# cube1324/ppo.c

Hardware: AMD Instinct MI355X
Metric: PPO updates/sec + env-steps/sec on 4096×256 synthetic rollout, 1/2/4/8 MI355X (higher is better)
Workload: dtype fp32

## Files before the change

include/ppo_ext.h:

```cpp
#ifndef PPO_EXT_H
#define PPO_EXT_H

#include <stddef.h>
#include <stdint.h>

#ifdef __cplusplus
extern "C" {
#endif


int         ppo_device_count(void);
int         ppo_set_device(int device);
const char* ppo_last_error(void);
void        ppo_clear_error(void);
void        ppo_synchronize(void);
const char* ppo_build_info(void);
int         ppo_struct_sizes(long* out, int n);

void* ppo_dev_alloc(size_t bytes);
void  ppo_dev_free(void* p);
void  ppo_h2d(void* dst, const void* src, size_t bytes);
void  ppo_d2h(void* dst, const void* src, size_t bytes);
void  ppo_d2d(void* dst, const void* src, size_t bytes);
void  ppo_dev_memset(void* dst, int value, size_t bytes);
// ... 23 lines not shown

void ppo_read_stats(void* ppo, double* out, int n);
void ppo_reset_stats(void* ppo);

int    ppo_set_max_grad_norm(void* ppo, float max_norm);
float  ppo_get_max_grad_norm(void* ppo);
double ppo_grad_norm_device(const float* d_a, long na, const float* d_b, long nb);

int    ppo_set_target_kl(void* ppo, float target_kl);
float  ppo_get_target_kl(void* ppo);
int    ppo_kl_history(void* ppo, double* out, int n);
int    ppo_policy_kl_device(const float* d_mu, const float* d_log_std, const float* d_action, const float* d_old_lp,
                            int m, int A, float eps, double* out2);
int    ppo_set_value_clip(void* ppo, float eps_v);
float  ppo_get_value_clip(void* ppo);
int    ppo_value_clip_old_values(void* ppo, const float* d_v_old, long n);
int    ppo_value_clip_head_device(const float* d_y, const float* d_v_old, const int* d_rows, const float* d_tgt, int m,
                                  float eps_v, float* d_g, double* out3);
int    ppo_set_obs_norm(void* ppo, float clip);
float  ppo_get_obs_norm(void* ppo);
int    ppo_obs_norm_freeze(void* ppo, int frozen);
int    ppo_obs_norm_fold_buffer(void* ppo);
int    ppo_obs_norm_get_state(void* ppo, double* out, long n);
int    ppo_obs_norm_set_state(void* ppo, const double* in, long n);
int    ppo_obs_norm_affine(void* ppo, float* mean, float* rstd, int S);
int    ppo_obs_normalize_device(void* ppo, const float* d_in, float* d_out, long m);
int    ppo_obs_stats_device(const float* d_x, long n, int S, double* out);
long ppo_gae_state(double* welford, float* v, float* v_next, long n);
void ppo_set_step_limit(void* ppo, long max_value_steps, long max_policy_steps);

void ppo_sample_action_device(void* policy, float* d_state, float* d_action, float* d_log_prob, int m,
                              unsigned long long seed, unsigned long long offset);

void ppo_fill_synthetic(void* ppo, int n_envs, int horizon, unsigned long long seed, float p_terminate);

void ppo_rollout_device(void* ppo, int n_envs, int horizon, int env_kind, unsigned long long seed);

int ppo_nn_input_rows(void* nn, float* out, int m);

int ppo_set_compute_dtype(void* ppo, int dtype);
int nn_set_compute_dtype(void* nn, int dtype);

int    ppo_gemm_tune(int force_cfg, int splitk_target);
int    ppo_gemm_flags(int flags);
double ppo_bench_gemm(int op, int m, int n, int l, int iters, int cfg);
double ppo_bench_streams(int two, int steps, int B, int out);
int    ppo_gemm16_tune(int force_cfg);
double ppo_bench_gemm16(int op, int m, int n, int l, int iters, int cfg, int splitk_target);

int    ppo_gemm_f32_engine(int engine);
int    ppo_gemm16_dma(int on);
int    ppo_gemm16_tn_width(int bn);
int    ppo_gemm_x3_tune(int force_cfg, int splitk_target);
int    ppo_x3_stamps(unsigned long long* out, int n);
int    ppo_g16_stamps(unsigned long long* out, int n);
double ppo_bench_gemm_x3(int op, int m, int n, int l, int iters, int cfg, int splitk_target);

enum { PPO_K_GEMM = 0, PPO_K_GAE = 1, PPO_K_ADAM = 2, PPO_K_GATHER = 3, PPO_K_HEAD = 4,
       PPO_K_COMM = 5, PPO_K_OTHER = 6, PPO_K_COUNT = 7 };
void ppo_prof_enable(int stride);
void ppo_prof_reset(void);
void ppo_prof_read(double* out_ms, double* out_work, long* out_launches);
void ppo_prof_kernel_events(int on);
int  ppo_prof_shapes(long long* keys, double* ms, long* launches, double* work, int cap);
int  ppo_prof_shape_issued(const long long* keys, long* issued, int n);
void ppo_prof_counts(long* out_total);
void ppo_prof_issued_work(double* out_work);

#ifdef __cplusplus
}
#endif
#endif
```

ppo.c_amd/csrc/gemm_x3.hip:

```cpp
#include "dev.h"
#include "vclip.h"

#include <algorithm>
#include <type_traits>

namespace {

typedef float f32x4 __attribute__((ext_vector_type(4)));
typedef float f32x16 __attribute__((ext_vector_type(16)));
typedef unsigned u32x4 __attribute__((ext_vector_type(4)));
typedef unsigned u32x2 __attribute__((ext_vector_type(2)));
typedef short s16x4 __attribute__((ext_vector_type(4)));
typedef short s16x8 __attribute__((ext_vector_type(8)));
typedef __bf16 bf16x8 __attribute__((ext_vector_type(8)));

constexpr int BK = 16;
enum { OP_NT = 0, OP_NN = 1, OP_TN = 2 };

__device__ unsigned long long g_x3_stamps[8192 * 8];

struct X3Args {
    const float* A; const float* B; float* C;
    int M, N, K, lda, ldb, ldc;
    const float* bias; int relu;
    const int* ridx; float* acopy;
    unsigned* bits_out; const unsigned* bits_in; int wpr;
    float* gbias;
    int kchunk, splits, tiles_m, tiles_n;
    float* slab;
    const float* ydot;
    float* ypart;
    const float* fold_g;
    const float* fold_w;
    const unsigned* fold_bits;
    int fold_wpr;
    float* fold_gw;
    const float* vh_ypart; const float* vh_b; const float* vh_t;
    float* vh_y; float* vh_gb; float* vh_loss;
    int vh_slots;
    PhipVClip vh_vc;
    const float* red_slab; float* red_out;
    long red_n, red_stride;
    int red_splits, red_wgs, gemm_wgs;
    hipEvent_t ev_start, ev_stop;
};

template <int NTH>
__device__ __forceinline__ void x3_slab_reduce_block(const X3Args& a, int blk, float* part) {
    typedef float f32x4_ __attribute__((ext_vector_type(4)));
    constexpr int Q = 4, C = NTH / Q;
    const int c = threadIdx.x % C, q = threadIdx.x / C;
    const long n4 = (a.red_n + 3) >> 2, s4 = a.red_stride >> 2;
    const long i = (long)blk * C + c;
    const int per = (a.red_splits + Q - 1) / Q;
    const int s0 = q * per, s1 = min(a.red_splits, s0 + per);
    const f32x4_* __restrict__ sv = reinterpret_cast<const f32x4_*>(a.red_slab);
    f32x4_ acc = {0.f, 0.f, 0.f, 0.f};
    if (i < n4) {
#pragma unroll 8
        for (int sp = s0; sp < s1; ++sp) acc += sv[(long)sp * s4 + i];
    }
    f32x4_* pv = reinterpret_cast<f32x4_*>(part);
    if (q) pv[(q - 1) * C + c] = acc;
    __syncthreads();
    if (q == 0 && i < n4) {
#pragma unroll
        for (int v = 0; v < Q - 1; ++v) acc += pv[v * C + c];
        if (4 * i + 4 <= a.red_n) {
            reinterpret_cast<f32x4_*>(a.red_out)[i] = acc;
        } else {
            for (int e = 0; e < 4; ++e)
                if (4 * i + e < a.red_n) a.red_out[4 * i + e] = acc[e];
        }
    }
}

__device__ __forceinline__ unsigned pack2(float lo, float hi) {
    typedef __bf16 bf16x2 __attribute__((ext_vector_type(2)));
    bf16x2 p = {(__bf16)lo, (__bf16)hi};
    return __builtin_bit_cast(unsigned, p);
}
__device__ __forceinline__ float bf_lo(unsigned u) { return __builtin_bit_cast(float, u << 16); }
__device__ __forceinline__ float bf_hi(unsigned u) { return __builtin_bit_cast(float, u & 0xffff0000u); }

__device__ __forceinline__ unsigned pack2_opaque(float lo, float hi) {
    unsigned u = pack2(lo, hi);
    asm("" : "+v"(u));
    return u;
}

__device__ __forceinline__ void split4(f32x4 f, u32x2& p0, u32x2& p1, u32x2& p2) {
    const unsigned a0 = pack2_opaque(f[0], f[1]), b0 = pack2_opaque(f[2], f[3]);
    const float r0 = f[0] - bf_lo(a0), r1 = f[1] - bf_hi(a0);
    const float r2 = f[2] - bf_lo(b0), r3 = f[3] - bf_hi(b0);
    const unsigned a1 = pack2_opaque(r0, r1), b1 = pack2_opaque(r2, r3);
    p0 = u32x2{a0, b0};
// ... 256 lines not shown
                }
                if (BITS && r < 16) {
                    const int row = r0 + (r & 3) + 8 * (r >> 2);
                    if (row < a.M && c0 < a.N) a.bits_out[(long)row * a.wpr + (c0 >> 5)] = word;
                }
            }
            if constexpr (YD) ydot_block(yp, i);
        }
    };
    if (OP == OP_NT && a.bits_out) body(std::true_type{});
    else body(std::false_type{});
}

template <int OP, int BM, int BN, int WARPS_M, int NTH, int OCC, int KG, int ABL = 0, int FOLD = 0, int KB = BK>
__device__ __forceinline__ void x3_body(const X3Args& a, int b, int grid) {
    constexpr int NTG = NTH / KG;
    constexpr int NW = NTG / 64, WARPS_N = NW / WARPS_M;
    constexpr int WM = BM / WARPS_M, WN = BN / WARPS_N;
    constexpr int TM = WM / 32, TN = WN / 32;
    static_assert(TM >= 1 && TN >= 1 && WARPS_M * WARPS_N == NW, "wave tiling");
    static_assert(KG == 1 || OP == OP_TN, "k-groups: grad_W only");
    constexpr bool A_MN = OP == OP_TN, B_MN = OP != OP_NT;
    using SA = StageX3<BM, A_MN, NTG, KB>;
    using SB = StageX3<BN, B_MN, NTG, KB>;
    constexpr int BUF = SA::SIZE + SB::SIZE;
    constexpr int KH = KB / 16;

    constexpr int NS = 3;
    extern __shared__ __attribute__((aligned(16))) unsigned short lds[];

    if constexpr (OP == OP_NN) {
        if (a.red_wgs && b >= a.gemm_wgs) {
            x3_slab_reduce_block<NTH>(a, b - a.gemm_wgs, reinterpret_cast<float*>(lds));
            return;
        }
    }

    const int nwg = (OP == OP_NN && a.red_wgs) ? a.gemm_wgs : grid;
    const int xcd = b & 7, qq = nwg >> 3, rr = nwg & 7;
    const int t = (xcd < rr ? xcd * (qq + 1) : rr * (qq + 1) + (xcd - rr) * qq) + (b >> 3);
    const int tn = t % a.tiles_n;
    const int rest = t / a.tiles_n;
    const int tm = rest % a.tiles_m;
    const int m0 = tm * BM, n0 = tn * BN;
    const int kbeg = (rest / a.tiles_m) * a.kchunk;
    const int kend = min(a.K, kbeg + a.kchunk);

    const int tid = threadIdx.x, lane = tid & 63;
    const int grp = KG > 1 ? __builtin_amdgcn_readfirstlane(tid / NTG) : 0;
    const int lt = KG > 1 ? tid % NTG : tid;
    const int w = lt >> 6;
    const int wm = w / WARPS_N, wn = w % WARPS_N;
    auto stamp = [&](int slot) {
        if (tid == 0 && b < 8192) {
            g_x3_stamps[b * 8 + slot] = __builtin_amdgcn_s_memtime();
            if (slot == 0 || slot == 3) g_x3_stamps[b * 8 + 4 + slot / 3] = __builtin_amdgcn_s_memrealtime();
        }
    };
    if (ABL & 32) stamp(0);
    const int r = lane & 31, h = lane >> 5;

    f32x16 acc[TM][TN];
#pragma unroll
    for (int i = 0; i < TM; ++i)
#pragma unroll
        for (int j = 0; j < TN; ++j)
#pragma unroll
            for (int e = 0; e < 16; ++e) acc[i][j][e] = 0.f;

    SA sa;
    SB sb;
    sa.init(a.A, a.lda, OP == OP_NT ? a.ridx : nullptr, m0, a.M, lt);
    sb.init(a.B, a.ldb, nullptr, n0, a.N, lt);
    constexpr bool syn = OP != OP_NT && FOLD != 0;
    constexpr int FMA_ = !syn ? 0 : OP == OP_NN ? 2 : 1;
    constexpr int FMB_ = syn ? 1 : 0;
    const float* fold_g = a.fold_g;
    if constexpr (OP == OP_TN && FOLD != 0) {
        if (a.vh_ypart) {
            float* gl = reinterpret_cast<float*>(lds + KG * NS * BUF);
            const bool head = tm == 0 && tn == 0;
            const float bias = a.vh_b[0];
            float ls = 0.f, sgs = 0.f;
            int nclip = 0, nrow = 0;
            for (int rr = tid; rr < kend - kbeg; rr += NTH) {
                const int row = kbeg + rr;
                float yv = 0.f;
                for (int q = 0; q < a.vh_slots; ++q) yv += a.vh_ypart[(long)q * a.K + row];
                yv += bias;
                float gv;
                const float lv = ppo::value_head_row(yv, a.vh_t[row], (float)a.K, a.vh_vc, row, gv, nclip);
                gl[rr] = gv;
                if (head) {
                    a.vh_y[row] = yv;
                    const_cast<float*>(a.fold_g)[row] = gv;
                    ls += lv;
                    sgs += gv;
                    ++nrow;
                }
            }
            if (head) {
                ls = ppo::wave_sum64(ls);
                sgs = ppo::wave_sum64(sgs);
                if (lane == 0) {
                    atomicAdd(a.vh_gb, sgs);
                    if (a.vh_loss) atomicAdd(a.vh_loss, ls * (1.0f / (float)a.K));
                }
                if (a.vh_vc.v_old) {
                    const float fc = ppo::wave_sum64((float)nclip), fr = ppo::wave_sum64((float)nrow);
// ... 324 lines not shown
                        wv[e] = a.bits_in[(long)min(r0 + (e & 3) + 8 * (e >> 2), a.M - 1) * a.wpr + (c0 >> 5)];
#pragma unroll
                    for (int e = 0; e < 16; ++e) keep[e] = (wv[e] >> r) & 1u;
                } else {
#pragma unroll
                    for (int e = 0; e < 16; ++e) keep[e] = true;
                }
            }
            unsigned word = 0;
#pragma unroll
            for (int e = 0; e < 16; ++e) {
                const int row = r0 + (e & 3) + 8 * (e >> 2);
                const bool ok = col_ok && row < a.M;
                float v = acc[i][j][e];
                if (OP == OP_TN && syn) v *= a.fold_w[row < a.M ? row : a.M - 1];
                float* dst = a.C + (long)row * a.ldc + col;
                if (OP == OP_NT) {
                    v += bcol;
                    if (a.relu) v = v > 0.f ? v : 0.f;
#ifdef PPO_X3_NTSTORE
                    if (ok) __builtin_nontemporal_store(v, dst);
#else
                    if (ok) *dst = v;
#endif
                    if (a.bits_out) {
                        const unsigned long long bb = __ballot(ok && v > 0.f);
                        if (r == e) word = h ? (unsigned)(bb >> 32) : (unsigned)bb;
                    }
                } else if (OP == OP_NN) {
#ifdef PPO_X3_NTSTORE
                    if (ok) __builtin_nontemporal_store(keep[e] ? v : 0.f, dst);
#else
                    if (ok) *dst = keep[e] ? v : 0.f;
#endif
                } else if (ok) {
                    if (a.slab) a.slab[(long)(kbeg / a.kchunk) * a.M * a.N + (long)row * a.N + col] = v;
                    else if (a.splits > 1) atomicAdd(dst, v);
                    else *dst = v;
                }
            }
            if (OP == OP_NT && a.bits_out && r < 16) {
                const int row = r0 + (r & 3) + 8 * (r >> 2);
                if (row < a.M && c0 < a.N) a.bits_out[(long)row * a.wpr + (c0 >> 5)] = word;
            }
        }
    if (ABL & 32) stamp(3);
}

template <int OP, int BM, int BN, int WARPS_M, int NTH, int OCC, int KG, int ABL = 0, int FOLD = 0, int KB = BK>
__global__ __launch_bounds__(NTH, OCC) void gemm_x3_kernel(X3Args a) {
    x3_body<OP, BM, BN, WARPS_M, NTH, OCC, KG, ABL, FOLD, KB>(a, (int)blockIdx.x, (int)gridDim.x);
}

#ifdef PPO_X3_DIAG
int g_x3_ablate = -1;
#endif

int g_x3_last_slots = 0;

template <int OP, int BM, int BN, int WARPS_M, int NTH, int OCC, int KG, int ABL = 0, int FOLD = 0, int KB = BK>
void launch_x3(X3Args a) {
    a.tiles_m = ppo_divup(a.M, BM);
    a.tiles_n = ppo_divup(a.N, BN);
    g_x3_last_slots = a.tiles_n * (NTH / KG / 64 / WARPS_M);
    if (a.splits < 1) a.splits = 1;
    long grid = (long)a.tiles_m * a.tiles_n * a.splits;
    PPO_REQUIRE(grid > 0 && grid < (1L << 31), "gemm_x3: grid out of range");
    if (a.red_wgs) {
        a.red_wgs = (int)ppo_divup((a.red_n + 3) / 4, NTH / 4);
        PPO_REQUIRE(OP == OP_NN && NTH >= 256 && grid + a.red_wgs < (1L << 31), "gemm_x3: carried reduce");
        a.gemm_wgs = (int)grid;
        grid += a.red_wgs;
    }
    PPO_REQUIRE(a.kchunk % (KG * KB) == 0 || a.splits == 1, "gemm_x3: split-K chunk vs k-groups");
    using SA = StageX3<BM, OP == OP_TN, NTH / KG, KB>;
    using SB = StageX3<BN, OP != OP_NT, NTH / KG, KB>;
    constexpr size_t lds0 = (size_t)KG * 3 * sizeof(unsigned short) * (SA::SIZE + SB::SIZE);
    static_assert(lds0 <= 160 * 1024, "gemm_x3: LDS images exceed 160 KiB");
    size_t lds = lds0;
    if (OP == OP_TN && FOLD && a.vh_ypart) {
        if (lds + 4 * (size_t)a.kchunk <= 160 * 1024) {
            lds += 4 * (size_t)a.kchunk;
        } else {
            phip_value_head(a.vh_ypart, a.vh_slots, a.vh_b, a.vh_t, a.K, a.vh_y, const_cast<float*>(a.fold_g), a.vh_gb,
                            a.vh_loss, &a.vh_vc);
            a.vh_ypart = nullptr;
        }
    }
    auto kern = gemm_x3_kernel<OP, BM, BN, WARPS_M, NTH, OCC, KG, ABL, FOLD, KB>;
    if (lds > 64 * 1024) {
        static bool attr = false;
        if (!attr) {
            PPO_CHECK(hipFuncSetAttribute((const void*)kern, hipFuncAttributeMaxDynamicSharedMemorySize, 160 * 1024));
            attr = true;
        }
    }
    if (a.ev_start || a.ev_stop)
        hipExtLaunchKernelGGL(kern, dim3((unsigned)grid), dim3(NTH), lds, ppo::stream(), a.ev_start, a.ev_stop, 0, a);
    else
        PPO_TIMED_LAUNCH(kern, dim3((unsigned)grid), dim3(NTH), lds, ppo::stream(), a);
    PPO_LAUNCH_CHECK();
}

template <int Q>
__global__ __launch_bounds__(256) void slab_reduce_kernel(const float* __restrict__ slab, float* __restrict__ out,
                                                          long n, long stride, int splits) {
    constexpr int C = 256 / Q;
    __shared__ f32x4 part[Q - 1][C];
    const int c = threadIdx.x % C, q = threadIdx.x / C;
    const long n4 = (n + 3) >> 2, s4 = stride >> 2;
    const long i = (long)blockIdx.x * C + c;
    const int per = (splits + Q - 1) / Q;
    const int s0 = q * per, s1 = min(splits, s0 + per);
    const f32x4* __restrict__ sv = reinterpret_cast<const f32x4*>(slab);
    f32x4 acc = {0.f, 0.f, 0.f, 0.f};
    if (i < n4) {
#pragma unroll 8
        for (int s = s0; s < s1; ++s) acc += sv[(long)s * s4 + i];
    }
    if (q) part[q - 1][c] = acc;
    __syncthreads();
    if (q == 0 && i < n4) {
#pragma unroll
        for (int v = 0; v < Q - 1; ++v) acc += part[v][c];
        if (4 * i + 4 <= n) {
            reinterpret_cast<f32x4*>(out)[i] = acc;
        } else {
            for (int e = 0; e < 4; ++e)
                if (4 * i + e < n) out[4 * i + e] = acc[e];
        }
    }
}

struct CfgX3 { int bm, bn, kg, slots_per_cu, kb; };
constexpr CfgX3 kCfgX3[] = {{256, 256, 1, 1, 16}, {128, 128, 1, 2, 16}, {128, 128, 1, 1, 16}, {128, 128, 2, 1, 16},
                            {64, 64, 1, 4, 16},   {256, 128, 1, 1, 16}, {64, 64, 1, 2, 32}};
int g_force_x3 = -1;
int g_split_x3 = 0;

template <int OP>
void launch_cfg_x3(int c, const X3Args& a) {
    if (a.ydot || a.fold_g) {
        switch (c) {
            case 0: launch_x3<OP, 256, 256, 4, 512, 2, 1, 0, 1>(a); return;
            case 2: launch_x3<OP, 128, 128, 4, 512, 2, 1, 0, 1>(a); return;
            case 4: launch_x3<OP, 64, 64, 2, 256, 4, 1, 0, 1>(a); return;
            case 5: launch_x3<OP, 256, 128, 4, 512, 2, 1, 0, 1>(a); return;
            case 6: launch_x3<OP, 64, 64, 2, 256, 2, 1, 0, 1, 32>(a); return;
            case 3:
                if constexpr (OP == OP_TN) { launch_x3<OP, 128, 128, 2, 512, 2, 2, 0, 1>(a); return; }
                [[fallthrough]];
            default: launch_x3<OP, 128, 128, 2, 256, 2, 1, 0, 1>(a); return;
        }
// ... 172 lines not shown
    PPO_REQUIRE(!fold_g || (fold_w && fold_gw && gb), "phip_x3_bwd_w: value-head fold operands");
    const int defer = ppo::g_defer_next;
    ppo::g_defer_next = 0;
    ppo::PendingReduce& pr = ppo::g_pending[phip_side_active() ? 1 : 0];
    PPO_REQUIRE(!pr.on, "phip_x3_bwd_w: a deferred split-K reduce was never run (phip_x3_defer_reduce without grad_x)");
    const int c = pick_x3(l, n, OP_TN);
    const long tiles = (long)ppo_divup(l, kCfgX3[c].bm) * ppo_divup(n, kCfgX3[c].bn);
    const int kq = kCfgX3[c].kb * kCfgX3[c].kg;
    const int target = g_split_x3 > 0 ? g_split_x3 : 256 * kCfgX3[c].slots_per_cu;
    int splits = (int)(target / tiles);
    const int max_splits = m / (8 * kq) > 0 ? m / (8 * kq) : 1;
    splits = std::max(1, std::min(splits, max_splits));
    int kchunk = m > 0 ? ppo_divup(ppo_divup(m, splits), kq) * kq : kq;
    splits = m > 0 ? ppo_divup(m, kchunk) : 1;
    const bool use_slab = splits > 1 && kchunk <= 1024 && al16(gW);
    ppo::ProfScope ps(PPO_K_GEMM, 2.0 * m * n * l, ppo::gemm_key(2, 1, m, n, l));
    if (m <= 0) {
        if (!zeroed) {
            phip_memset(gW, 0, sizeof(float) * (size_t)l * n);
            if (gb) phip_memset(gb, 0, sizeof(float) * (size_t)l);
        }
        return;
    }
    X3Args a{};
    a.A = g; a.lda = l; a.B = x; a.ldb = n; a.C = gW; a.ldc = n;
    a.M = l; a.N = n; a.K = m; a.kchunk = kchunk; a.splits = splits;
    a.gbias = gb;
    a.fold_g = fold_g; a.fold_w = fold_w; a.fold_gw = fold_gw;
    a.vh_ypart = ypart; a.vh_slots = slots; a.vh_b = b; a.vh_t = tgt; a.vh_y = y; a.vh_gb = gb_out; a.vh_loss = loss_accum;
    if (vc) a.vh_vc = *vc;
    if (splits > 1 && !zeroed) {
        if (!use_slab) phip_memset(gW, 0, sizeof(float) * (size_t)l * n);
        if (gb) phip_memset(gb, 0, sizeof(float) * (size_t)l);
    }
    if (!use_slab) {
        launch_cfg_x3<OP_TN>(c, a);
        return;
    }
    a.slab = ppo::slab_scratch((size_t)splits * l * n);
    hipEvent_t e0 = nullptr, e1 = nullptr;
    const bool timed = ppo::take_kernel_events(&e0, &e1);
    a.ev_start = timed ? e0 : nullptr;
    if (defer && splits < 64) {
        a.ev_stop = timed ? e1 : nullptr;
        launch_cfg_x3<OP_TN>(c, a);
        pr = ppo::PendingReduce{a.slab, gW, (long)l * n, (long)l * n, splits, true};
        return;
    }
    a.ev_stop = nullptr;
    launch_cfg_x3<OP_TN>(c, a);
    ppo::slab_reduce(a.slab, gW, (long)l * n, (long)l * n, splits, timed ? e1 : nullptr);
}

int ppo_gemm_x3_tune(int force_cfg, int splitk_target) {
    g_force_x3 = force_cfg;
    if (splitk_target >= 0) g_split_x3 = splitk_target;
    return (int)(sizeof(kCfgX3) / sizeof(kCfgX3[0]));
}

double ppo_bench_gemm_x3(int op, int m, int n, int l, int iters, int cfg, int splitk_target) {
    ppo::ensure_device();
    const size_t sx = (size_t)m * n, sw = (size_t)l * n, sy = (size_t)m * l;
    float* x = (float*)phip_malloc(4 * sx);
    float* W = (float*)phip_malloc(4 * sw);
    float* y = (float*)phip_malloc(4 * sy);
    float* b = (float*)phip_malloc(4 * (size_t)std::max(l, n));
    float* gw = (float*)phip_malloc(4 * sw);
    unsigned* bits = (unsigned*)phip_malloc(4 * (size_t)m * ppo_divup(std::max(l, n), 32));
    phip_fill_uniform(x, (long)sx, 1, -1.f, 1.f);
    phip_fill_uniform(W, (long)sw, 2, -0.1f, 0.1f);
    phip_fill_uniform(y, (long)sy, 3, -1.f, 1.f);
    phip_fill_uniform(b, (long)std::max(l, n), 4, -0.1f, 0.1f);
    phip_memset(bits, 0xff, 4 * (size_t)m * ppo_divup(std::max(l, n), 32));
    const int saved = g_force_x3, saved_split = g_split_x3;
    g_force_x3 = cfg;
    g_split_x3 = splitk_target;
    float* fold = (op >= 4) ? (float*)phip_malloc(4 * ((size_t)m * (2 * ppo_divup(l, 64) + 1) + (size_t)l)) : nullptr;
    if (fold) phip_fill_uniform(fold, (long)m * (2 * ppo_divup(l, 64) + 1) + l, 5, -0.1f, 0.1f);
    auto run = [&]() {
        if (op == 0) phip_x3_fwd(y, x, nullptr, nullptr, W, b, m, n, l, 1, bits);
        else if (op == 3) phip_x3_fwd(y, x, nullptr, nullptr, W, b, m, n, l, 0, nullptr);
        else if (op == 1) phip_x3_bwd_x(x, y, W, bits, m, n, l);
        else if (op == 4) phip_x3_fwd_vhead(y, x, nullptr, nullptr, W, b, m, n, l, 1, bits, fold, fold + l);
        else if (op == 5) phip_x3_bwd_x_fold(x, nullptr, bits, fold, fold + m, W, bits, m, n, l);
        else if (op == 6) phip_x3_bwd_w_fold(gw, b, y, fold, fold + m, fold + m + l, x, m, n, l, 0);
        else phip_x3_bwd_w(gw, b, y, x, m, n, l, 0);
    };
    for (int i = 0; i < 3; ++i) run();
    hipEvent_t e0, e1;
    PPO_CHECK(hipEventCreate(&e0));
    PPO_CHECK(hipEventCreate(&e1));
    PPO_CHECK(hipEventRecord(e0, ppo::stream()));
    for (int i = 0; i < iters; ++i) run();
    PPO_CHECK(hipEventRecord(e1, ppo::stream()));
    PPO_CHECK(hipEventSynchronize(e1));
    float ms = 0.f;
    PPO_CHECK(hipEventElapsedTime(&ms, e0, e1));
    PPO_CHECK(hipEventDestroy(e0));
    PPO_CHECK(hipEventDestroy(e1));
    g_force_x3 = saved;
    g_split_x3 = saved_split;
    phip_free(x); phip_free(W); phip_free(y); phip_free(b); phip_free(gw); phip_free(bits); phip_free(fold);
    return 1000.0 * ms / (iters > 0 ? iters : 1);
}

int ppo_x3_stamps(unsigned long long* out, int n) {
    phip_sync();
    PPO_CHECK(hipMemcpyFromSymbol(out, HIP_SYMBOL(g_x3_stamps), sizeof(unsigned long long) * (size_t)std::min(n, 8192 * 8)));
    return 8192 * 8;
}

}
```

ppo.c_amd/csrc/ppo_hip.h:

```cpp
#ifndef PPO_HIP_H
#define PPO_HIP_H

#include <stddef.h>
#include <stdint.h>

#ifdef __cplusplus
extern "C" {
#endif

void  phip_init(void);
void* phip_malloc(size_t bytes);
void  phip_free(void* p);
void  phip_h2d(void* dst, const void* src, size_t bytes);
void  phip_d2h(void* dst, const void* src, size_t bytes);
void  phip_d2d(void* dst, const void* src, size_t bytes);
void  phip_memset(void* dst, int value, size_t bytes);
void  phip_sync(void);
void  phip_side_fork(void);
void  phip_side_use(int on);
int   phip_comm_inline(void);
int   phip_side_active(void);
void  phip_side_join(void);
void  phip_record_error(const char* msg);
void  phip_drain(void);

typedef struct {
    const float* v_old;
    const int* rows;
    float eps;
    unsigned long long* counts;
} PhipVClip;

void phip_linear_fwd(float* y, const float* x, const float* W, const float* b, int m, int n, int l, int relu);
void phip_linear_fwd_bits(float* y, const float* x, const float* W, const float* b, int m, int n, int l, int relu,
                          unsigned* bits);
void phip_linear_bwd_x(float* gx, const float* g, const float* W, const float* mask, int m, int n, int l);
void phip_linear_fwd_gather(float* y, const float* x, const int* ridx, float* xcopy, const float* W, const float* b,
                            int m, int n, int l, int relu, unsigned* bits);
void phip_linear_bwd_x_bits(float* gx, const float* g, const float* W, const float* mask, const unsigned* bits, int m,
                            int n, int l);
void phip_linear_bwd_w(float* gW, float* gb, const float* g, const float* x, int m, int n, int l);
void phip_linear_bwd_pair(float* gW, float* gb, float* gx, const float* g, const float* x, const float* W,
                          const unsigned* bits, int m, int n, int l, int zeroed);
void phip_linear_bwd_w_ex(float* gW, float* gb, const float* g, const float* x, int m, int n, int l, int zeroed);

void phip_linear16_fwd(void* y, int ty, const void* x, int tx, const int* ridx, void* xcopy16, const void* W16,
                       const float* b, int m, int n, int l, int relu, unsigned* bits);
void phip_linear16_bwd_x(void* gx, int tgx, const void* g, int tg, const void* W16, const unsigned* bits, int m,
                         int n, int l);
void phip_linear16_bwd_w(float* gW, float* gb, const void* g, int tg, const void* x, int tx, int m, int n, int l,
                         int zeroed);
int  phip_x3_supported(int op, int m, int n, int l);
void phip_x3_fwd(float* y, const float* x, const int* ridx, float* xcopy, const float* W, const float* b, int m,
                 int n, int l, int relu, unsigned* bits);
void phip_x3_defer_reduce(int on);
void phip_x3_bwd_x(float* gx, const float* g, const float* W, const unsigned* bits, int m, int n, int l);
void phip_x3_bwd_w(float* gW, float* gb, const float* g, const float* x, int m, int n, int l, int zeroed);
int  phip_x3_fwd_vhead(float* y, const float* x, const int* ridx, float* xcopy, const float* W, const float* b, int m,
                       int n, int l, int relu, unsigned* bits, const float* ydot, float* ypart);
void phip_x3_bwd_x_fold(float* gx, const float* g, const unsigned* fold_bits, const float* fold_g, const float* fold_w,
                        const float* W, const unsigned* bits, int m, int n, int l);
void phip_x3_bwd_w_fold(float* gW, float* gb, const float* h, const float* fold_g, const float* fold_w, float* fold_gw,
                        const float* x, int m, int n, int l, int zeroed);
void phip_x3_bwd_w_vhead(float* gW, float* gb, const float* h, float* fold_g, const float* fold_w, float* fold_gw,
                         const float* x, int m, int n, int l, int zeroed, const float* ypart, int slots, const float* b,
                         const float* tgt, float* y, float* gb_out, float* loss_accum, const PhipVClip* vc);
void phip_gather_rows_bf16(unsigned short* dst, const float* src, const int* rows, int m, int S);
void phip_f32_to_bf16(unsigned short* dst, const float* src, long count);

void phip_rollout_rows(int* rows, int E, int T);
void phip_env_reset(int kind, float* env_state, float* state, int E, int T, int S, uint64_t seed);
void phip_env_first_obs(int kind, const float* env_state, float* state, int E, int T, int S);
void phip_sample_rows(const float* mu, const float* log_std, const int* rows, float* action, float* logprob, int E,
                      int A, uint64_t seed, uint64_t step);
void phip_env_step(int kind, float* env_state, float* state, const float* action, float* next_state, float* reward,
                   uint8_t* term, uint8_t* trunc, int E, int T, int t, int S, int A, uint64_t seed);

typedef struct {
    int L;
    int sizes[9];
    int relu[8];
    long woff[8], boff[8];
    float *params, *grads, *m, *v;
    long span;
    float *log_std, *log_std_grad, *m_ls, *v_ls;
    float* wt; long wt_cap;
} PhipTinyNet;
typedef struct {
    int policy;
    const float *state, *action, *logprob, *adv, *adv_target;
    int limit, B, num_batches, n_epochs;
    long max_steps;
    const int* perms;
    uint32_t feistel_k[64];
    const float *steps, *steps_ls;
    float b1, b2, eps, ent_coeff;
    float* stats;
} PhipTinyPhase;
int phip_tiny_update(const PhipTinyNet* net, const PhipTinyPhase* ph);
int phip_cluster_update(const PhipTinyNet* net, const PhipTinyPhase* ph);
int phip_cluster_error(void);
void phip_cluster_report(void);
int phip_cluster_deep_update(const PhipTinyNet* net, const PhipTinyPhase* ph);
unsigned* phip_cluster_err_dev(void);

void phip_relu(float* x, long count);
void phip_relu_bwd(const float* y, float* g, long count);
void phip_axpy(float* y, const float* x, long count);
void phip_mse(const float* y, const float* t, long count, float* grad, float* d_loss, float* d_loss_accum);
void phip_mse_vclip(const float* y, const float* t, long count, float* grad, float* d_loss_accum, const PhipVClip* vc);
// ... 155 lines not shown
```

ppo.c_amd/host/neural_network.c:

```c
#include "internal.h"

#include <math.h>
#include <stdint.h>
#include <stdlib.h>
#include <string.h>

int nn_is_relu(const NeuralNetwork* nn, int layer) {
    const ActivationFunction* a = nn->layers[layer].d_activation_function;
    return a && a->activation != NULL;
}

static NeuralNetwork** g_nets = NULL;
static int g_nets_n = 0, g_nets_cap = 0;

static void nn_registry_add(NeuralNetwork* nn) {
    if (g_nets_n == g_nets_cap) {
        g_nets_cap = g_nets_cap ? 2 * g_nets_cap : 16;
        NeuralNetwork** p = (NeuralNetwork**)realloc(g_nets, sizeof(NeuralNetwork*) * (size_t)g_nets_cap);
        if (!p) die("host allocation failed");
        g_nets = p;
    }
    g_nets[g_nets_n++] = nn;
}

// ... 319 lines not shown
    if (top == L && nn_is_relu(nn, L - 1)) {
        float* top = nn->layers[L].d_grad_x;
        if (top != d_grad_out) phip_d2d(top, d_grad_out, sizeof(float) * (size_t)m * nn->output_size);
        phip_relu_bwd(nn->layers[L].d_input, top, (long)m * nn->output_size);
        g = top;
    }
    if (!grads_zero) phip_memset(nn->d_grads, 0, sizeof(float) * (size_t)nn->num_params);
    if (nn->dtype == 1) {
        if (nn->bits_m != m) die("nn_backward_dev (bf16): backward must follow a forward over the same rows");
        int tg = top == L ? 0 : 1;
        long hi = nn->num_params + (reduce_extra > 0 ? reduce_extra : 0);
        for (int i = top - 1; i >= 0; i--) {
            Layer* ly = &nn->layers[i];
            const void* x = i == 0 ? (const void*)nn->d_x0 : (const void*)ly->d_input;
            phip_linear16_bwd_w(ly->d_grad_weights, ly->d_grad_biases, g, tg, x, i == 0 ? nn->x0_dtype : 1, m,
                                ly->input_size, ly->output_size, 1);
            int tgx = tg;
            if (i > 0 || want_grad_x0) {
                const int relu_in = i > 0 && nn_is_relu(nn, i - 1);
                tgx = i > 0 ? 1 : 0;
                phip_linear16_bwd_x(ly->d_grad_x, tgx, g, tg, nn->d_w16 + nn->param_offset[i],
                                    relu_in ? act_bits(nn, i) : NULL, m, ly->input_size, ly->output_size);
            }
            g = ly->d_grad_x;
            tg = tgx;
            if (reduce_extra >= 0) bucket_flush(nn, i, &hi);
        }
        nn->cache_m_backward = m;
        return;
    }
    long hi = nn->num_params + (reduce_extra > 0 ? reduce_extra : 0);
    for (int i = top - 1; i >= 0; i--) {
        Layer* ly = &nn->layers[i];
        const float* x = i == 0 ? nn->d_x0 : ly->d_input;
        const int n = ly->input_size, l = ly->output_size;
        const int want_gx = i > 0 || want_grad_x0;
        const int relu_in = i > 0 && nn_is_relu(nn, i - 1);
        const unsigned* bits = relu_in && nn->bits_m == m ? act_bits(nn, i) : NULL;
        if (fold && i == top - 1) {
            const float* h = nn->layers[i + 1].d_input;
            phip_x3_defer_reduce(want_gx);
            phip_x3_bwd_w_vhead(ly->d_grad_weights, ly->d_grad_biases, h, fold->g, fold->w, fold->gw_out, x, m, n, l, 1,
                                fold->ypart, fold->slots, fold->b, fold->tgt, fold->y, fold->gb, fold->loss, fold->vc);
            if (want_gx) {
                if (relu_in && !bits) die("nn_value_fold_step: the forward's ReLU′ bits are missing");
                phip_x3_bwd_x_fold(ly->d_grad_x, NULL, act_bits(nn, i + 1), fold->g, fold->w, ly->d_weights, bits, m, n,
                                   l);
            }
        } else if (i == L - 1 && want_gx && (!relu_in || bits) &&
            phip_out_bwd_wide(ly->d_grad_weights, ly->d_grad_biases, ly->d_grad_x, g, x, ly->d_weights, relu_in, m, n,
                              l)) {
        } else if (use_x3_layer(m, n, l) && phip_x3_supported(2, m, n, l)) {
            const int pair = want_gx && (!relu_in || bits);
            phip_x3_defer_reduce(pair);
            phip_x3_bwd_w(ly->d_grad_weights, ly->d_grad_biases, g, x, m, n, l, 1);
            if (pair) phip_x3_bwd_x(ly->d_grad_x, g, ly->d_weights, bits, m, n, l);
            else if (want_gx) phip_linear_bwd_x_bits(ly->d_grad_x, g, ly->d_weights, ly->d_input, NULL, m, n, l);
        } else if (want_gx && (!relu_in || bits)) {
            phip_linear_bwd_pair(ly->d_grad_weights, ly->d_grad_biases, ly->d_grad_x, g, x, ly->d_weights, bits, m, n,
                                 l, 1);
        } else {
            phip_linear_bwd_w_ex(ly->d_grad_weights, ly->d_grad_biases, g, x, m, n, l, 1);
            if (want_gx)
                phip_linear_bwd_x_bits(ly->d_grad_x, g, ly->d_weights, relu_in ? ly->d_input : NULL, NULL, m, n, l);
        }
        g = ly->d_grad_x;
        if (reduce_extra >= 0) bucket_flush(nn, i, &hi);
    }
    nn->cache_m_backward = m;
}

int nn_out_head_ok(const NeuralNetwork* nn, int head) {
    const char* e = getenv("PPO_OUT_HEAD");
    if ((e && e[0] == '0') || phip_gemm_deterministic()) return 0;
    const int L = nn->num_layers - 1;
    if (L < 2 || nn_is_relu(nn, L - 1)) return 0;
    if (nn->dtype == 1 && (head != 0 || nn->param_offset[L - 1] % 8 != 0)) return 0;
    return phip_out_head_supported(head, nn->layers[L - 1].input_size, nn->layers[L - 1].output_size);
}

void nn_out_head_step(NeuralNetwork* nn, int head, const float* d_x, const int* d_rows, float* d_xcopy, int m,
                      int grads_zero, long reduce_extra, const float* tgt, const float* log_std, const float* action,
                      const float* adv, const float* old_lp, float eps, float ent_coeff, float* grad_log_std,
                      float* loss_accum, const PhipVClip* vc) {
    const int L = nn->num_layers - 1;
    nn_forward_dev_upto(nn, d_x, d_rows, d_xcopy, m, L - 1, NULL);
    nn_ensure_grad(nn, m);
    if (!grads_zero) phip_memset(nn->d_grads, 0, sizeof(float) * (size_t)nn->num_params);
    Layer* ly = &nn->layers[L - 1];
    const int b16 = nn->dtype == 1;

    phip_out_head(head, b16, ly->d_input, nn_is_relu(nn, L - 2), b16 ? (const void*)(nn->d_w16 + nn->param_offset[L - 1])
                                                                     : (const void*)ly->d_weights,
                  ly->d_biases, m, ly->input_size, ly->output_size, tgt, log_std, action, adv, old_lp, eps, ent_coeff,
                  nn->layers[L].d_input, ly->d_grad_x, ly->d_grad_weights, ly->d_grad_biases, grad_log_std,
                  loss_accum, vc);
    nn->d_output = nn->layers[L].d_input;
    nn_backward_dev_top(nn, ly->d_grad_x, m, 0, 1, reduce_extra, L - 1, NULL);
}

int nn_value_fold_ok(const NeuralNetwork* nn, int m) {
    const char* e = getenv("PPO_VALUE_FOLD");
    if ((e && e[0] == '0') || phip_gemm_deterministic()) return 0;
    const int L = nn->num_layers - 1;
    if (nn->dtype != 0 || L < 2 || nn->output_size != 1 || nn_is_relu(nn, L - 1) || !nn_is_relu(nn, L - 2)) return 0;
    const Layer* hid = &nn->layers[L - 2];
// ... 252 lines not shown
```

ppo.c_amd/ppo_ffi.py:

```python
import ctypes as C
import os

HERE = os.path.dirname(os.path.abspath(__file__))
LIB_PATH = os.path.join(HERE, "lib", "libppo.so")

c_float_p = C.POINTER(C.c_float)
c_int_p = C.POINTER(C.c_int)
c_bool_p = C.POINTER(C.c_bool)
c_long_p = C.POINTER(C.c_long)
VOIDFN = C.c_void_p


class ActivationFunction(C.Structure):
    _fields_ = [("activation", C.c_void_p), ("activation_derivative", C.c_void_p)]


class Layer(C.Structure):
    _fields_ = [(n, c_float_p) for n in ("weights", "biases", "grad_weights", "grad_biases", "input",
                                          "d_weights", "d_biases", "d_grad_weights", "d_grad_biases",
                                          "d_input", "d_grad_x")] + [
        ("activation_function", C.POINTER(ActivationFunction)),
        ("d_activation_function", C.POINTER(ActivationFunction)),
        ("input_size", C.c_int), ("output_size", C.c_int)]

# ... 27 lines not shown
class TrajectoryBuffer(C.Structure):
    pass


TrajectoryBuffer._fields_ = (
    [(n, c_bool_p if "terminated" in n or "truncated" in n else c_float_p) for n in _BUF_PTRS]
    + [("h_" + n, c_bool_p if "terminated" in n or "truncated" in n else c_float_p) for n in _BUF_PTRS]
    + [("d_" + n, c_bool_p if "terminated" in n or "truncated" in n else c_float_p) for n in _BUF_PTRS]
    + [("random_idx", c_int_p), ("state_size", C.c_int), ("action_size", C.c_int), ("capacity", C.c_int),
       ("idx", C.c_int), ("full", C.c_bool)]
    + [(n, VOIDFN) for n in ("state", "action", "next_state", "reward", "logprob", "advantage", "adv_target",
                             "terminated", "truncated")]
    + [("h_random_idx", c_int_p), ("on_device", C.c_int), ("random_idx_is_device", C.c_int)])


class Adam(C.Structure):
    _fields_ = [("weights", C.POINTER(c_float_p)), ("grad_weights", C.POINTER(c_float_p)), ("lengths", c_int_p),
                ("m", c_float_p), ("v", c_float_p), ("beta1", C.c_float), ("beta2", C.c_float),
                ("time_step", C.c_int), ("size", C.c_int), ("num_layers", C.c_int),
                ("on_device", C.c_int), ("flat", C.c_int), ("grad_scale", C.c_float), ("span", C.c_long)]


class PPO(C.Structure):
    _fields_ = [("buffer", C.POINTER(TrajectoryBuffer)), ("policy", C.POINTER(GaussianPolicy)),
                ("V", C.POINTER(NeuralNetwork)), ("adam_policy", C.POINTER(Adam)), ("adam_V", C.POINTER(Adam)),
                ("adam_entropy", C.POINTER(Adam)), ("lambda_", C.c_float), ("epsilon", C.c_float),
                ("ent_coeff", C.c_float), ("lr_policy", C.c_float), ("lr_V", C.c_float), ("use_cuda", C.c_bool),
                ("dev", C.c_void_p)]


class Env(C.Structure):
    _fields_ = [("free_env", VOIDFN), ("reset_env", VOIDFN), ("step_env", VOIDFN), ("state_size", C.c_int),
                ("action_size", C.c_int), ("horizon", C.c_int), ("gamma", C.c_float)]


STRUCTS = [Layer, NeuralNetwork, GaussianPolicy, TrajectoryBuffer, Adam, PPO, Env]

_P = C.c_void_p
_F = c_float_p
_SIGS = {
    "ppo_device_count": (C.c_int, []),
    "ppo_set_device": (C.c_int, [C.c_int]),
    "ppo_last_error": (C.c_char_p, []),
    "ppo_synchronize": (None, []),
    "ppo_gemm_tune": (C.c_int, [C.c_int, C.c_int]),
    "ppo_gemm16_tune": (C.c_int, [C.c_int]),
    "ppo_gemm_flags": (C.c_int, [C.c_int]),
    "ppo_bench_gemm16": (C.c_double, [C.c_int] * 7),
    "ppo_gemm_f32_engine": (C.c_int, [C.c_int]),
    "ppo_gemm16_dma": (C.c_int, [C.c_int]),
    "ppo_gemm16_tn_width": (C.c_int, [C.c_int]),
    "ppo_gemm_x3_tune": (C.c_int, [C.c_int, C.c_int]),
    "ppo_bench_gemm_x3": (C.c_double, [C.c_int] * 7),
    "ppo_x3_stamps": (C.c_int, [C.POINTER(C.c_ulonglong), C.c_int]),
    "ppo_g16_stamps": (C.c_int, [C.POINTER(C.c_ulonglong), C.c_int]),
    "ppo_set_compute_dtype": (C.c_int, [_P, C.c_int]),
    "ppo_rollout_device": (None, [_P, C.c_int, C.c_int, C.c_int, C.c_ulonglong]),
    "nn_set_compute_dtype": (C.c_int, [_P, C.c_int]),
    "ppo_bench_gemm": (C.c_double, [C.c_int] * 6),
    "ppo_bench_streams": (C.c_double, [C.c_int] * 4),
    "ppo_build_info": (C.c_char_p, []),
    "ppo_struct_sizes": (C.c_int, [c_long_p, C.c_int]),
    "ppo_dev_alloc": (_P, [C.c_size_t]),
    "ppo_dev_free": (None, [_P]),
    "ppo_h2d": (None, [_P, _P, C.c_size_t]),
    "ppo_d2h": (None, [_P, _P, C.c_size_t]),
    "ppo_d2d": (None, [_P, _P, C.c_size_t]),
    "ppo_dev_memset": (None, [_P, C.c_int, C.c_size_t]),
    "ppo_comm_unique_id": (C.c_int, [C.c_char_p, C.c_int]),
    "ppo_comm_init": (C.c_int, [C.c_int, C.c_int, C.c_char_p]),
    "ppo_comm_rank": (C.c_int, []),
    "ppo_comm_world": (C.c_int, []),
    "ppo_comm_finalize": (None, []),
    "ppo_comm_allreduce_f32": (None, [_P, C.c_long]),
    "ppo_welford_combine": (None, [_P, C.c_int, _P]),
    "ppo_comm_loopback_peers": (C.c_int, [_P, _P, C.c_int]),
    "ppo_comm_loopback_peer_grads": (C.c_int, [_P, _P, C.c_long]),
    "ppo_comm_loopback_clear": (None, []),
    "ppo_comm_loopback_peer_hash": (C.c_int, [_P, C.c_int]),
    "ppo_comm_mode": (C.c_char_p, []),
    "ppo_comm_check_replicas": (C.c_int, [_P]),
    "ppo_param_hash": (C.c_ulonglong, [_P]),
    "ppo_clear_error": (None, []),
    "ppo_nn_input_rows": (C.c_int, [_P, _P, C.c_int]),
    "ppo_gae_state": (C.c_long, [_P, _P, _P, C.c_long]),
    "ppo_comm_barrier": (None, []),
    "ppo_comm_max_f64": (C.c_double, [C.c_double]),
    "ppo_update": (None, [_P, C.c_float, C.c_int, C.c_int, C.c_int, C.c_int, C.c_ulonglong]),
    "ppo_read_stats": (None, [_P, C.POINTER(C.c_double), C.c_int]),
    "ppo_reset_stats": (None, [_P]),
    "ppo_set_step_limit": (None, [_P, C.c_long, C.c_long]),
    "ppo_set_max_grad_norm": (C.c_int, [_P, C.c_float]),
    "ppo_get_max_grad_norm": (C.c_float, [_P]),
    "ppo_grad_norm_device": (C.c_double, [_P, C.c_long, _P, C.c_long]),
    "ppo_set_target_kl": (C.c_int, [_P, C.c_float]),
    "ppo_get_target_kl": (C.c_float, [_P]),
    "ppo_kl_history": (C.c_int, [_P, C.POINTER(C.c_double), C.c_int]),
    "ppo_policy_kl_device": (C.c_int, [_P, _P, _P, _P, C.c_int, C.c_int, C.c_float, C.POINTER(C.c_double)]),
    "ppo_set_value_clip": (C.c_int, [_P, C.c_float]),
    "ppo_get_value_clip": (C.c_float, [_P]),
    "ppo_value_clip_old_values": (C.c_int, [_P, _P, C.c_long]),
    "ppo_value_clip_head_device": (C.c_int, [_P, _P, _P, _P, C.c_int, C.c_float, _P, C.POINTER(C.c_double)]),
    "ppo_set_obs_norm": (C.c_int, [_P, C.c_float]),
    "ppo_get_obs_norm": (C.c_float, [_P]),
    "ppo_obs_norm_freeze": (C.c_int, [_P, C.c_int]),
    "ppo_obs_norm_fold_buffer": (C.c_int, [_P]),
# ... 157 lines not shown
```

Measured before the change: 3.487 million.

## Fuse x3 backward weight-grad, input-grad and pending slab reduce into one launch

Adds a combined backward kernel whose grid is partitioned among the input-gradient GEMM (NN), the split-K weight-gradient GEMM (TN), and the previous layer's deferred split-K slab reduction. The neural-network backward pass uses it by default for paired layers, replacing two or three separate launches. The goal is to cut launch overhead and let the independent GEMMs fill the device together. In exchange, both GEMMs share one LDS size and launch bounds, and the path is skipped for small split-K chunks, so coverage depends on shape.

```diff
diff --git a/include/ppo_ext.h b/include/ppo_ext.h
--- a/include/ppo_ext.h
+++ b/include/ppo_ext.h
@@ -99,6 +99,11 @@
 int    ppo_gemm16_dma(int on);
 int    ppo_gemm16_tn_width(int bn);
 int    ppo_gemm_x3_tune(int force_cfg, int splitk_target);
+int    ppo_x3_bwd_layer(int fused, float* gW, float* gb, float* gx, const float* g, const float* x, const float* W,
+                        const unsigned* bits, int m, int n, int l, const float* red_slab, float* red_out, long red_n,
+                        int red_splits);
+int    ppo_x3_bwd_fused_default(void);
+void   ppo_x3_slab_reduce(const float* slab, float* out, long n, int splits);
 int    ppo_x3_stamps(unsigned long long* out, int n);
 int    ppo_g16_stamps(unsigned long long* out, int n);
 double ppo_bench_gemm_x3(int op, int m, int n, int l, int iters, int cfg, int splitk_target);
diff --git a/ppo.c_amd/csrc/gemm_x3.hip b/ppo.c_amd/csrc/gemm_x3.hip
--- a/ppo.c_amd/csrc/gemm_x3.hip
+++ b/ppo.c_amd/csrc/gemm_x3.hip
@@ -42,6 +42,7 @@
     const float* red_slab; float* red_out;
     long red_n, red_stride;
     int red_splits, red_wgs, gemm_wgs;
+    int stamp_base;
     hipEvent_t ev_start, ev_stop;
 };
 
@@ -404,9 +405,10 @@
     const int w = lt >> 6;
     const int wm = w / WARPS_N, wn = w % WARPS_N;
     auto stamp = [&](int slot) {
-        if (tid == 0 && b < 8192) {
-            g_x3_stamps[b * 8 + slot] = __builtin_amdgcn_s_memtime();
-            if (slot == 0 || slot == 3) g_x3_stamps[b * 8 + 4 + slot / 3] = __builtin_amdgcn_s_memrealtime();
+        const int sb = b + a.stamp_base;
+        if (tid == 0 && sb < 8192) {
+            g_x3_stamps[sb * 8 + slot] = __builtin_amdgcn_s_memtime();
+            if (slot == 0 || slot == 3) g_x3_stamps[sb * 8 + 4 + slot / 3] = __builtin_amdgcn_s_memrealtime();
         }
     };
     if (ABL & 32) stamp(0);
@@ -837,6 +839,22 @@
     x3_body<OP, BM, BN, WARPS_M, NTH, OCC, KG, ABL, FOLD, KB>(a, (int)blockIdx.x, (int)gridDim.x);
 }
 
+template <int ABL = 0>
+__global__ __launch_bounds__(512, 2) void gemm_x3_bwd_fused_kernel(X3Args ax, X3Args aw) {
+    const int b = (int)blockIdx.x;
+    if (b < ax.gemm_wgs) {
+        x3_body<OP_NN, 256, 256, 4, 512, 2, 1, ABL>(ax, b, ax.gemm_wgs);
+        return;
+    }
+    const int bw = b - ax.gemm_wgs;
+    if (bw < aw.gemm_wgs) {
+        x3_body<OP_TN, 128, 128, 2, 512, 2, 2, ABL>(aw, bw, aw.gemm_wgs);
+        return;
+    }
+    extern __shared__ __attribute__((aligned(16))) unsigned short lds[];
+    x3_slab_reduce_block<512>(ax, bw - aw.gemm_wgs, reinterpret_cast<float*>(lds));
+}
+
 #ifdef PPO_X3_DIAG
 int g_x3_ablate = -1;
 #endif
@@ -884,6 +902,38 @@
         hipExtLaunchKernelGGL(kern, dim3((unsigned)grid), dim3(NTH), lds, ppo::stream(), a.ev_start, a.ev_stop, 0, a);
     else
         PPO_TIMED_LAUNCH(kern, dim3((unsigned)grid), dim3(NTH), lds, ppo::stream(), a);
+    PPO_LAUNCH_CHECK();
+}
+
+template <int ABL = 0>
+void launch_x3_bwd_fused(X3Args ax, X3Args aw) {
+    ax.tiles_m = ppo_divup(ax.M, 256);
+    ax.tiles_n = ppo_divup(ax.N, 256);
+    aw.tiles_m = ppo_divup(aw.M, 128);
+    aw.tiles_n = ppo_divup(aw.N, 128);
+    if (aw.splits < 1) aw.splits = 1;
+    const long tx = (long)ax.tiles_m * ax.tiles_n, tw = (long)aw.tiles_m * aw.tiles_n * aw.splits;
+    if (ax.red_wgs) ax.red_wgs = (int)ppo_divup((ax.red_n + 3) / 4, 512 / 4);
+    const long grid = tx + tw + ax.red_wgs;
+    PPO_REQUIRE(tx > 0 && tw > 0 && grid < (1L << 31), "gemm_x3 (fused backward): grid out of range");
+    PPO_REQUIRE(aw.kchunk % 32 == 0 || aw.splits == 1, "gemm_x3 (fused backward): split-K chunk vs k-groups");
+    ax.gemm_wgs = (int)tx;
+    aw.gemm_wgs = (int)tw;
+    aw.stamp_base = (int)tx;
+    using XA = StageX3<256, false, 512>;
+    using XB = StageX3<256, true, 512>;
+    using WA = StageX3<128, true, 256>;
+    constexpr size_t lds_x = (size_t)3 * sizeof(unsigned short) * (XA::SIZE + XB::SIZE);
+    constexpr size_t lds_w = (size_t)2 * 3 * sizeof(unsigned short) * (2 * WA::SIZE);
+    constexpr size_t lds = lds_x > lds_w ? lds_x : lds_w;
+    static_assert(lds <= 160 * 1024, "gemm_x3 (fused backward): LDS images exceed 160 KiB");
+    auto kern = gemm_x3_bwd_fused_kernel<ABL>;
+    static bool attr = false;
+    if (!attr) {
+        PPO_CHECK(hipFuncSetAttribute((const void*)kern, hipFuncAttributeMaxDynamicSharedMemorySize, 160 * 1024));
+        attr = true;
+    }
+    PPO_TIMED_LAUNCH(kern, dim3((unsigned)grid), dim3(512), lds, ppo::stream(), ax, aw);
     PPO_LAUNCH_CHECK();
 }
 
@@ -1162,6 +1212,88 @@
     ppo::slab_reduce(a.slab, gW, (long)l * n, (long)l * n, splits, timed ? e1 : nullptr);
 }
 
+constexpr bool kX3FusedDefault = true;
+
+static int x3_bwd_fused(float* gW, float* gb, float* gx, const float* g, const float* x, const float* W,
+                        const unsigned* bits, int m, int n, int l, int zeroed) {
+    if (m <= 0 || n <= 0 || l <= 0) return 0;
+    if (!(gW && gx && g && x && W && n % 4 == 0 && l % 4 == 0 && al16(g) && al16(x) && al16(W))) return 0;
+    if (pick_x3(m, n, OP_NN) != 0) return 0;
+    const CfgX3 cw = kCfgX3[3];
+    const long tiles = (long)ppo_divup(l, cw.bm) * ppo_divup(n, cw.bn);
+    const int kq = cw.kb * cw.kg;
+    const int target = g_split_x3 > 0 ? g_split_x3 : 256 * cw.slots_per_cu;
+    int splits = (int)(target / tiles);
+    const int max_splits = m / (8 * kq) > 0 ? m / (8 * kq) : 1;
+    splits = std::max(1, std::min(splits, max_splits));
+    const int kchunk = ppo_divup(ppo_divup(m, splits), kq) * kq;
+    splits = ppo_divup(m, kchunk);
+    if (splits > 1 && kchunk <= 1024 && al16(gW) && g_force_x3 < 0) return 0;
+    ppo::g_defer_next = 0;
+    ppo::ProfScope ps(PPO_K_GEMM, 4.0 * m * n * l, ppo::gemm_key(3, 1, m, n, l));
+    X3Args ax{};
+    ax.A = g; ax.lda = l; ax.B = W; ax.ldb = n; ax.C = gx; ax.ldc = n;
+    ax.M = m; ax.N = n; ax.K = l; ax.kchunk = l; ax.splits = 1;
+    ax.bits_in = bits; ax.wpr = ppo_divup(n, 32);
+    ppo::PendingReduce& pr = ppo::g_pending[phip_side_active() ? 1 : 0];
+    if (pr.on) {
+        ax.red_slab = pr.slab; ax.red_out = pr.out; ax.red_n = pr.n; ax.red_stride = pr.stride;
+        ax.red_splits = pr.splits; ax.red_wgs = 1;
+        pr.on = false;
+    }
+    X3Args aw{};
+    aw.A = g; aw.lda = l; aw.B = x; aw.ldb = n; aw.C = gW; aw.ldc = n;
+    aw.M = l; aw.N = n; aw.K = m; aw.kchunk = kchunk; aw.splits = splits;
+    aw.gbias = gb;
+    if (splits > 1 && !zeroed) {
+        phip_memset(gW, 0, sizeof(float) * (size_t)l * n);
+        if (gb) phip_memset(gb, 0, sizeof(float) * (size_t)l);
+    }
+#ifdef PPO_X3_DIAG
+    if (g_x3_ablate < 0) {
+        const char* e = getenv("PPO_X3_ABLATE");
+        g_x3_ablate = e ? atoi(e) : 0;
+    }
+    if (g_x3_ablate == 32) { launch_x3_bwd_fused<32>(ax, aw); return 1; }
+#endif
+    launch_x3_bwd_fused<0>(ax, aw);
+    return 1;
+}
+
+int phip_x3_bwd_fused(float* gW, float* gb, float* gx, const float* g, const float* x, const float* W,
+                      const unsigned* bits, int m, int n, int l, int zeroed) {
+    if (kX3FusedDefault == ((ppo_gemm_flags(-1) & 64) != 0)) return 0;
+    return x3_bwd_fused(gW, gb, gx, g, x, W, bits, m, n, l, zeroed);
+}
+
+int ppo_x3_bwd_fused_default(void) { return kX3FusedDefault ? 1 : 0; }
+
+int ppo_x3_bwd_layer(int fused, float* gW, float* gb, float* gx, const float* g, const float* x, const float* W,
+                     const unsigned* bits, int m, int n, int l, const float* red_slab, float* red_out, long red_n,
+                     int red_splits) {
+    ppo::ensure_device();
+    ppo::PendingReduce& pr = ppo::g_pending[phip_side_active() ? 1 : 0];
+    PPO_REQUIRE(!pr.on, "ppo_x3_bwd_layer: a deferred split-K reduce is pending");
+    if (fused && !red_slab) return x3_bwd_fused(gW, gb, gx, g, x, W, bits, m, n, l, 0);
+    if (red_slab) PPO_REQUIRE(red_out && red_n > 0 && red_n % 4 == 0 && red_splits >= 1 && red_splits < 64 &&
+                              al16(red_slab) && al16(red_out), "ppo_x3_bwd_layer: carried reduce operands");
+    if (fused) {
+        pr = ppo::PendingReduce{red_slab, red_out, red_n, red_n, red_splits, true};
+        const int ran = x3_bwd_fused(gW, gb, gx, g, x, W, bits, m, n, l, 0);
+        pr.on = false;
+        return ran;
+    }
+    phip_x3_bwd_w(gW, gb, g, x, m, n, l, 0);
+    if (red_slab) pr = ppo::PendingReduce{red_slab, red_out, red_n, red_n, red_splits, true};
+    phip_x3_bwd_x(gx, g, W, bits, m, n, l);
+    return 1;
+}
+
+void ppo_x3_slab_reduce(const float* slab, float* out, long n, int splits) {
+    ppo::ensure_device();
+    ppo::slab_reduce(slab, out, n, n, splits, nullptr);
+}
+
 int ppo_gemm_x3_tune(int force_cfg, int splitk_target) {
     g_force_x3 = force_cfg;
     if (splitk_target >= 0) g_split_x3 = splitk_target;
@@ -1187,7 +1319,13 @@
     g_split_x3 = splitk_target;
     float* fold = (op >= 4) ? (float*)phip_malloc(4 * ((size_t)m * (2 * ppo_divup(l, 64) + 1) + (size_t)l)) : nullptr;
     if (fold) phip_fill_uniform(fold, (long)m * (2 * ppo_divup(l, 64) + 1) + l, 5, -0.1f, 0.1f);
+    float* gx = (op == 7 || op == 8) ? (float*)phip_malloc(4 * sx) : nullptr;
     auto run = [&]() {
+        if (op == 7) { phip_x3_bwd_w(gw, b, y, x, m, n, l, 1); phip_x3_bwd_x(gx, y, W, bits, m, n, l); return; }
+        if (op == 8) {
+            PPO_REQUIRE(x3_bwd_fused(gw, b, gx, y, x, W, bits, m, n, l, 1), "ppo_bench_gemm_x3: no fused launch at this shape");
+            return;
+        }
         if (op == 0) phip_x3_fwd(y, x, nullptr, nullptr, W, b, m, n, l, 1, bits);
         else if (op == 3) phip_x3_fwd(y, x, nullptr, nullptr, W, b, m, n, l, 0, nullptr);
         else if (op == 1) phip_x3_bwd_x(x, y, W, bits, m, n, l);
@@ -1210,7 +1348,7 @@
     PPO_CHECK(hipEventDestroy(e1));
     g_force_x3 = saved;
     g_split_x3 = saved_split;
-    phip_free(x); phip_free(W); phip_free(y); phip_free(b); phip_free(gw); phip_free(bits); phip_free(fold);
+    phip_free(x); phip_free(W); phip_free(y); phip_free(b); phip_free(gw); phip_free(bits); phip_free(fold); phip_free(gx);
     return 1000.0 * ms / (iters > 0 ? iters : 1);
 }
 
diff --git a/ppo.c_amd/csrc/ppo_hip.h b/ppo.c_amd/csrc/ppo_hip.h
--- a/ppo.c_amd/csrc/ppo_hip.h
+++ b/ppo.c_amd/csrc/ppo_hip.h
@@ -56,6 +56,8 @@
 void phip_x3_defer_reduce(int on);
 void phip_x3_bwd_x(float* gx, const float* g, const float* W, const unsigned* bits, int m, int n, int l);
 void phip_x3_bwd_w(float* gW, float* gb, const float* g, const float* x, int m, int n, int l, int zeroed);
+int  phip_x3_bwd_fused(float* gW, float* gb, float* gx, const float* g, const float* x, const float* W,
+                       const unsigned* bits, int m, int n, int l, int zeroed);
 int  phip_x3_fwd_vhead(float* y, const float* x, const int* ridx, float* xcopy, const float* W, const float* b, int m,
                        int n, int l, int relu, unsigned* bits, const float* ydot, float* ypart);
 void phip_x3_bwd_x_fold(float* gx, const float* g, const unsigned* fold_bits, const float* fold_g, const float* fold_w,
diff --git a/ppo.c_amd/host/neural_network.c b/ppo.c_amd/host/neural_network.c
--- a/ppo.c_amd/host/neural_network.c
+++ b/ppo.c_amd/host/neural_network.c
@@ -395,6 +395,12 @@
                               l)) {
         } else if (use_x3_layer(m, n, l) && phip_x3_supported(2, m, n, l)) {
             const int pair = want_gx && (!relu_in || bits);
+            if (pair && phip_x3_bwd_fused(ly->d_grad_weights, ly->d_grad_biases, ly->d_grad_x, g, x, ly->d_weights, bits,
+                                          m, n, l, 1)) {
+                g = ly->d_grad_x;
+                if (reduce_extra >= 0) bucket_flush(nn, i, &hi);
+                continue;
+            }
             phip_x3_defer_reduce(pair);
             phip_x3_bwd_w(ly->d_grad_weights, ly->d_grad_biases, g, x, m, n, l, 1);
             if (pair) phip_x3_bwd_x(ly->d_grad_x, g, ly->d_weights, bits, m, n, l);
diff --git a/ppo.c_amd/ppo_ffi.py b/ppo.c_amd/ppo_ffi.py
--- a/ppo.c_amd/ppo_ffi.py
+++ b/ppo.c_amd/ppo_ffi.py
@@ -103,6 +103,9 @@
     "ppo_gemm16_tn_width": (C.c_int, [C.c_int]),
     "ppo_gemm_x3_tune": (C.c_int, [C.c_int, C.c_int]),
     "ppo_bench_gemm_x3": (C.c_double, [C.c_int] * 7),
+    "ppo_x3_bwd_layer": (C.c_int, [C.c_int] + [_P] * 7 + [C.c_int] * 3 + [_P, _P, C.c_long, C.c_int]),
+    "ppo_x3_bwd_fused_default": (C.c_int, []),
+    "ppo_x3_slab_reduce": (None, [_P, _P, C.c_long, C.c_int]),
     "ppo_x3_stamps": (C.c_int, [C.POINTER(C.c_ulonglong), C.c_int]),
     "ppo_g16_stamps": (C.c_int, [C.POINTER(C.c_ulonglong), C.c_int]),
     "ppo_set_compute_dtype": (C.c_int, [_P, C.c_int]),
```

Result: no change. 3.493 million (median of 5 runs) (+0.2%).
